# mj-will/aspire

Measured on AMD Instinct MI355X. Metric: particle-steps/sec (N x n_steps), 1M particles d=32; log-evidence err vs ref, higher is better.
Workload: dtype f64

## Files before the change

### aspire_amd/csrc/asmc_common.h

```cpp
#pragma once
#include <hip/hip_runtime.h>
#include <stdint.h>
#include <stdio.h>
#include <string.h>

#include "../../include/asmc.h"

#define ASMC_WAVE 64
#define ASMC_BLOCK 256
#define ASMC_MAX_BLOCKS 2048
#define ASMC_SCAN_TILE 2048
#define ASMC_PCN_MAX_GRID (1 << 20)
#define ASMC_GAMMA_BATCH 8
#define ASMC_MAX_PCN_STEPS 2048
#define BM_SC_N 256
#define BM_LG_N 128
#define BM_TAB_N (BM_SC_N + BM_LG_N)

void asmc_set_error(const char* fmt, ...);
void asmc_bm_table_host(double* tab);
struct asmc_ctx;
int asmc_count_nonfinite_enqueue(asmc_ctx* ctx, int64_t n, const double* v, hipStream_t st);
unsigned long long* asmc_count_slot(asmc_ctx* ctx);
struct asmc_ctx;
// ... 30 lines not shown
            return ASMC_ERR_ARG;                                  \
        }                                                         \
    } while (0)

#define ASMC_LAUNCH_CHECK()                                                                 \
    do {                                                                                    \
        hipError_t _e = hipGetLastError();                                                  \
        if (_e != hipSuccess) {                                                             \
            asmc_set_error("kernel launch failed: %s (%s:%d)", hipGetErrorString(_e),       \
                           __FILE__, __LINE__);                                             \
            return ASMC_ERR_HIP;                                                            \
        }                                                                                   \
    } while (0)

#define ASMC_TILECTR_BYTES ((sizeof(unsigned int) * (2 * ASMC_MAX_PCN_STEPS + 4) + 255) / 256 * 256)
struct asmc_ctx {
    int device;
    int64_t n_max;
    int d_max;
    int num_cu;
    double* d_partials;
    double* d_small;
    unsigned long long* d_keys;
    double* d_tiles;
    long long* d_tiles_i;
    double* d_gram;
    unsigned int* d_guide;
    unsigned char* d_flags;
    double* d_gamma;
    int64_t gam_n;
// ... 22 lines not shown
    long long* d_counts;
    double* d_rho;
    unsigned long long* d_stretch;
    unsigned long long* d_mh;
    unsigned int* d_tilectr;
    unsigned int* d_bar;
    unsigned int bar_base[17];
    unsigned long long flow_nonfinite;
    int poison_lds;
    int isw_disabled;
    unsigned long long* d_pcgtab;
    long long* d_select;
    unsigned long long ptab_tag, ysplit_seq;
    double* d_ptab;
    double* d_bmtab;
    double* d_mmtab;
    double* d_f16tab;
    size_t f16tab_bytes;
    int (*count_hook)(void*, asmc_stream);
    void* count_hook_user;
    long long* count_cell;
    int count_cells;
    int64_t count_n_global;
    int mutate_defer, mutate_pending_steps;
    hipEvent_t ev_mutate;
    hipEvent_t ev_is;
    int is_result_pending;
    unsigned long long lq_nan;
    void* rccl_allreduce;
    void* rccl_comm;
// ... 83 lines not shown
```

### aspire_amd/csrc/asmc_ctx.hip

```cpp
#include <dlfcn.h>
#include <stdarg.h>

#include <math.h>

#include "asmc_common.h"

static thread_local char g_err[512] = "";

void asmc_set_error(const char* fmt, ...) {
    va_list ap;
    va_start(ap, fmt);
    vsnprintf(g_err, sizeof(g_err), fmt, ap);
    va_end(ap);
}

__global__ __launch_bounds__(256) void k_poison_lds(int words) {
    extern __shared__ unsigned int s_poison[];
    for (int i = threadIdx.x; i < words; i += 256) s_poison[i] = 0xFFFFFFFFu;
    __syncthreads();
    if (s_poison[(threadIdx.x * 977) % words] != 0xFFFFFFFFu) __builtin_trap();
}
void asmc_poison_lds(asmc_ctx* ctx, hipStream_t st) {
    const int bytes = 160 * 1024 - 1024;
    static bool attr_set_dev[ASMC_MAX_DEVICES] = {false}; bool& attr_set = attr_set_dev[asmc_dev_slot(ctx)];
// ... 170 lines not shown
    const size_t student = (size_t)d_max * (d_max + 1) + (size_t)(ASMC_STUDENT_MAX_ROWS / 64) * (d_max + 2);
    dmalloc((void**)&c->d_student, sizeof(double) * student);
    if (e == hipSuccess) e = hipHostMalloc((void**)&c->h_student, sizeof(double) * student, hipHostMallocDefault);
    dmalloc((void**)&c->d_counts, sizeof(long long) * (size_t)(ASMC_MAX_PCN_STEPS + ASMC_MAX_BLOCKS + n_max / 64 + 8));
    dmalloc((void**)&c->d_rho, sizeof(double) * (ASMC_MAX_PCN_STEPS + 8));
    dmalloc((void**)&c->d_stretch, sizeof(unsigned long long) * ASMC_MAX_PCN_STEPS);
    dmalloc((void**)&c->d_mh, sizeof(unsigned long long) * ASMC_MAX_PCN_STEPS);
    if (e == hipSuccess) e = hipMemset(c->d_tilectr, 0, ASMC_TILECTR_BYTES);
    dmalloc((void**)&c->d_bar, sizeof(unsigned int) * 1024 * 17);
    if (e == hipSuccess) e = hipMemset(c->d_bar, 0, sizeof(unsigned int) * 1024 * 17);
    dmalloc((void**)&c->d_pcgtab, sizeof(unsigned long long) * (64 * 4 + 8));
    dmalloc((void**)&c->d_select, sizeof(long long) * (2 * (ASMC_SELECT_THREADS / 64) + 8));
    dmalloc((void**)&c->d_ptab, sizeof(double) * (2 * 32 * 32 + 32 + 3 * ASMC_MAX_COMPONENTS * (1 + 2 * 32) + 64));
    dmalloc((void**)&c->d_bmtab, sizeof(double) * 2 * BM_TAB_N);
    dmalloc((void**)&c->d_ref, sizeof(double) * (128 + 128 * 128));
    if (e == hipSuccess) {
        double tab[2 * BM_TAB_N];
        asmc_bm_table_host(tab);
        e = hipMemcpy(c->d_bmtab, tab, sizeof(tab), hipMemcpyHostToDevice);
    }
    if (e == hipSuccess) e = hipHostMalloc((void**)&c->h_pinned, sizeof(double) * 8192, hipHostMallocDefault);
    if (e == hipSuccess) e = hipHostMalloc((void**)&c->h_gram, sizeof(double) * (128 + 128 * 128), hipHostMallocDefault);
    if (e != hipSuccess) {
        asmc_set_error("asmc_ctx_create: allocation failed: %s", hipGetErrorString(e));
        asmc_ctx_destroy(c);
        return ASMC_ERR_NOMEM;
    }
    *ctx_out = c;
    return ASMC_OK;
}
// ... 15 lines not shown
    if (c->h_student) (void)hipHostFree(c->h_student);
    if (c->d_ysoa) (void)hipFree(c->d_ysoa);
    if (c->d_xpad) (void)hipFree(c->d_xpad);
    (void)hipFree(c->d_counts);
    (void)hipFree(c->d_rho);
    (void)hipFree(c->d_stretch);
    (void)hipFree(c->d_mh);
    (void)hipFree(c->d_tilectr);
    (void)hipFree(c->d_rec);
    (void)hipFree(c->d_bar);
    (void)hipFree(c->d_pcgtab);
    (void)hipFree(c->d_select);
    (void)hipFree(c->d_ptab);
    (void)hipFree(c->d_bmtab);
    (void)hipFree(c->d_ref);
    if (c->prof_ev) {
        for (int i = 0; i < 2 * ASMC_PROF_MAX; i++) (void)hipEventDestroy(c->prof_ev[i]);
        delete[] c->prof_ev;
        delete[] c->prof_label;
    }
    if (c->h_pinned) (void)hipHostFree(c->h_pinned);
    if (c->h_gram) (void)hipHostFree(c->h_gram);
    if (c->ev_mutate) (void)hipEventDestroy(c->ev_mutate);
    if (c->ev_is) (void)hipEventDestroy(c->ev_is);
    delete c;
    return ASMC_OK;
}

}
```

### aspire_amd/csrc/asmc_flow_dev.h

```cpp
#pragma once
#include "asmc_common.h"

typedef float floatx16 __attribute__((ext_vector_type(16)));


__device__ __forceinline__ float flow_standardise(float x, float loc, float scale, float rcp) {
    const float a = x - loc;
    const float q0 = a * rcp;
    const float r = fmaf(-scale, q0, a);
    return fmaf(r, rcp, q0);
}

typedef float flow_std2 __attribute__((ext_vector_type(2)));
__device__ __forceinline__ flow_std2 flow_standardise2(flow_std2 x, flow_std2 loc, flow_std2 scale, flow_std2 rcp) {
    const flow_std2 a = x - loc;
    const flow_std2 q0 = a * rcp;
    const flow_std2 r = __builtin_elementwise_fma(-scale, q0, a);
    return __builtin_elementwise_fma(r, rcp, q0);
}

template <bool INVERSE>
__device__ __forceinline__ void flow_affine(float& x, float sraw, float t, float& ladj, int form) {
    if (form == 0) {
        const float sv = 2.0f - 4.0f * __builtin_amdgcn_rcpf(__expf(sraw) + 1.0f);
// ... 594 lines not shown
                for (int nb = 0; nb < NBM; nb++) ah[nb] = ahn[nb], al[nb] = aln[nb];
            } else {
                a_load(g + 1, ah, al);
            }
            __builtin_amdgcn_sched_barrier(0);
        }
    }
    flow_f2 lacc = {0.0f, 0.0f};
#pragma unroll
    for (int q = 0; q < H / 2; q += 2)
        flow_affine2<false>(trans[q], trans[q + 1], o[q / 16][q % 16], o[(q + 1) / 16][(q + 1) % 16], o[(H / 2 + q) / 16][(H / 2 + q) % 16],
                            o[(H / 2 + q + 1) / 16][(H / 2 + q + 1) % 16], lacc, FORM >= 0 ? FORM : form);
    ladj += lacc.x + lacc.y;
}

template <int H, int W, int THREADS>
__device__ __forceinline__ void flow_stage_hs(float* __restrict__ sp, const float* __restrict__ packed, int n_layers) {
    using FD = FlowDims<H, W>;
    constexpr int L4 = FD::LAYER / 4, B4 = FD::BIAS / 4;
    const int total4 = n_layers * L4;
    for (int i4 = threadIdx.x; i4 < total4; i4 += THREADS) {
        const int in_layer = i4 % L4;
        if (in_layer < B4) {
            reinterpret_cast<float4*>(sp)[i4] = reinterpret_cast<const float4*>(packed)[i4];
            continue;
        }
        const int local = in_layer - B4;
        if ((local / 64) & 1) continue;
        const float4 f0 = reinterpret_cast<const float4*>(packed)[i4], f1 = reinterpret_cast<const float4*>(packed)[i4 + 64];
        const float xv[8] = {f0.x, f0.y, f0.z, f0.w, f1.x, f1.y, f1.z, f1.w};
        half8 hi, lo;
        float wmax = 0.0f;
        split8_f16<false>(xv, hi, lo, wmax);
        reinterpret_cast<half8*>(sp)[i4] = hi;
        reinterpret_cast<half8*>(sp)[i4 + 64] = lo;
    }
}
```

### aspire_amd/csrc/asmc_pcn.hip

```cpp
#include <stdlib.h>

#include <chrono>

#include "asmc_common.h"
#include "asmc_tile.h"
#include "asmc_pcn_dev.h"
#include "asmc_transform_dev.h"

template <typename T>
__device__ __forceinline__ double mixture_eval(const MixDev& m, int d, const char* row) {
    double best = -INFINITY;
    double terms[ASMC_MAX_COMPONENTS];
    const int C = m.C;
    for (int c = 0; c < C; c++) {
        double q = 0.0;
        const double* mu = m.mu + (size_t)c * d;
        const double* pr = m.prec + (size_t)c * d;
        for (int j = 0; j < d; j++) {
            const double t = row_get<T>(row, j) - mu[j];
            q = fma(t * t, pr[j], q);
        }
        const double v = m.logw[c] - 0.5 * q;
        terms[c] = v;
        best = fmax(best, v);
// ... 2921 lines not shown
            pc.noise = ASMC_NOISE_F64;
            if (prm->x_dtype == ASMC_F64)
                return launch_pcn_step<double, 0>(ctx, n, (double*)x, ll, lp, lq, pc, d_rho, 0, d_block, &grid, nullptr, nullptr, nullptr, st);
            return launch_pcn_step<float, 0>(ctx, n, (float*)x, ll, lp, lq, pc, d_rho, 0, d_block, &grid, nullptr, nullptr, nullptr, st);
        };
        rc = convert(PCN_WHITEN);
        if (rc) return rc;
        const bool fused = soa && asmc_pcn_flow_fused_ok(prm, flow);
        if (d_noise > 0 && !fused) {
            asmc_set_error("asmc_pcn_mutate_flow: the zero-padded form needs the one-kernel step");
            return ASMC_ERR_UNSUPPORTED;
        }
        if (fused) {
            ASMC_HIP(hipMemsetAsync(ctx->d_tilectr, 0, ASMC_TILECTR_BYTES + ((size_t)((n + 63) / 64) + 15) / 16 * 16, st));
            pd.tile_par = ctx->d_flags;
        }
        for (int t = 0; t < (fused ? n_steps : 0); t++) {
            const uint32_t step = step0 + (uint32_t)t;
            rc = pcn_prepare_gamma(ctx, n, pd, step, st);
            if (rc) return rc;
            PcnAdaptArgs ad = {ctx->d_tilectr + ASMC_MAX_PCN_STEPS + t,
                               reinterpret_cast<unsigned long long*>(ctx->d_tilectr + 2 * ASMC_MAX_PCN_STEPS),
                               ctx->count_hook ? ctx->count_cell : nullptr,
                               ctx->count_hook && t > 0 ? ctx->count_cell : nullptr, d_counts, d_rho, d_rho_hist,
                               prm->target_accept, ctx->count_hook ? ctx->count_n_global : n, t, prm->adapt, t == n_steps - 1};
            const int lag = prm->adapt >= 2 ? prm->adapt : 1;
            if (ctx->count_hook && lag > ctx->count_cells) {
                asmc_set_error("adapt_lag %d needs %d exchange cells, the installed hook has %d (asmc_pcn_set_count_cells)", lag, lag, ctx->count_cells);
                return ASMC_ERR_ARG;
            }
// ... 344 lines not shown
```

### aspire_amd/csrc/asmc_pcn_dev.h

```cpp
#pragma once
#include "asmc_common.h"

bool asmc_flow_math_split();

struct PcnAdaptArgs {
    unsigned int* done;
    unsigned long long* nonfinite;
    long long* cell;
    const long long* prev_cell;
    long long* counts_out;
    double* rho;
    double* rho_hist;
    double target;
    int64_t n;
    int t, adapt;
    int last;
};

__device__ __forceinline__ double pcn_adapt_rho(double rho, long long c, int64_t n, double target, int t) {
    const double acc = (double)c / (double)n;
    double r = exp(log(rho) + (acc - target) / pow((double)(t + 1), 0.75));
    r = r < 1e-4 ? 1e-4 : r;
    r = r > 0.99 ? 0.99 : r;
    return r;
// ... 344 lines not shown
        return (double)__uint_as_float(v);
    }
}
template <typename T>
__device__ __forceinline__ void soa_store(__amdgpu_buffer_rsrc_t r, unsigned voff, unsigned soff, double x) {
    if constexpr (sizeof(T) == 8) {
        using u2 = decltype(__builtin_amdgcn_raw_buffer_load_b64(r, 0, 0, 0));
        __builtin_amdgcn_raw_buffer_store_b64(__builtin_bit_cast(u2, x), r, (int)voff, (int)soff, 0);
    } else {
        __builtin_amdgcn_raw_buffer_store_b32(__float_as_uint((float)x), r, (int)voff, (int)soff, 0);
    }
}


bool asmc_pcn_flow_fused_ok(const asmc_pcn_params* prm, const asmc_coupling* f);
int asmc_pcn_flow_fused_launch(asmc_ctx* ctx, int64_t n, int x_dtype, double* ll, double* lp, double* lq, const PcnDev& pd,
                               const asmc_coupling* f, const double* rho_ptr, uint32_t step, unsigned int* tile_counter,
                               long long* block_counts, int* grid_out, const PcnAdaptArgs& adapt, hipStream_t st);

#define MM_WHITEN 0
#define MM_STEP 1
#define MM_UNWHITEN 2
#define MM_STEP_T 3
#define MM_XPROPOSE 4
#define MM_XPROPOSE_T 5
#define MM_UNWHITEN_X 6
bool asmc_pcn_mm_supported(int d, const void* x);
int asmc_pcn_mm_pack(asmc_ctx* ctx, const PcnDev& pd, hipStream_t st);
int asmc_pcn_flow16_tables(asmc_ctx* ctx, const PcnDev& pd, const asmc_coupling* f, hipStream_t st);
int asmc_pcn_flow16_launch(asmc_ctx* ctx, int64_t n, int x_dtype, void* x, double* ll, double* lp, double* lq, const PcnDev& pd,
// ... 9 lines not shown
```

### aspire_amd/csrc/asmc_pcn_fused.hip

```cpp
#include <stdlib.h>

#include "asmc_common.h"
#include <type_traits>
#include "asmc_pcn_dev.h"
#include "asmc_flow_dev.h"

#ifndef FUSED_THREADS
#define FUSED_THREADS 512
#endif

#define FUSED_TL_DOUBLES 1368
#define FUSED_MAX_COMPONENTS 4
#ifndef MV_DEPTH
#define MV_DEPTH 4
#endif
typedef double double2v __attribute__((ext_vector_type(2)));
__host__ __device__ constexpr int mv_group(int bi) {
    int g = 0;
    while ((g + 1) * (g + 2) <= bi) g++;
    return g;
}
template <int I, int N, typename F>
__device__ __forceinline__ void mv_for_each(F& f) {
    if constexpr (I < N) {
// ... 16 lines not shown
    y = __builtin_bit_cast(double, ((unsigned long long)hi[1] << 32) | lo[1]);
}
__device__ __forceinline__ void fused_swap16(double& x, double& y) {
    const unsigned long long xb = __builtin_bit_cast(unsigned long long, x), yb = __builtin_bit_cast(unsigned long long, y);
    const auto lo = __builtin_amdgcn_permlane16_swap((unsigned)xb, (unsigned)yb, false, false);
    const auto hi = __builtin_amdgcn_permlane16_swap((unsigned)(xb >> 32), (unsigned)(yb >> 32), false, false);
    x = __builtin_bit_cast(double, ((unsigned long long)hi[0] << 32) | lo[0]);
    y = __builtin_bit_cast(double, ((unsigned long long)hi[1] << 32) | lo[1]);
}
__device__ __forceinline__ void fused_transpose4(double& q0, double& q1, double& q2, double& q3) {
    fused_swap32(q0, q2);
    fused_swap32(q1, q3);
    fused_swap16(q0, q1);
    fused_swap16(q2, q3);
}
#ifndef HS1P_PREFETCH
#define HS1P_PREFETCH false
#endif
#ifndef FUSED_PRIO_A
#define FUSED_PRIO_A 2
#define FUSED_PRIO_B 1
#endif
#ifndef MV_CHUNK
#define MV_CHUNK 8
#endif
template <typename T, int W, int NOISE, bool HS, int KIND = ASMC_FLOW_COUPLING, bool MIX = false>
__global__ __launch_bounds__(FUSED_THREADS) void k_pcn_flow_fused(
    int64_t n, double* __restrict__ ll, double* __restrict__ lp, double* __restrict__ lq, const double* __restrict__ ptab,
    PcnScalars p, const double* rho_ptr, uint32_t step, const float* __restrict__ packed, int n_layers,
    const float* __restrict__ loc, const float* __restrict__ scale, float ladj0, float base_const,
    unsigned int* __restrict__ tile_counter, long long* __restrict__ block_counts, PcnAdaptArgs ad, int par_words, int affine) {
    constexpr int D = 32, H = 16, THREADS = FUSED_THREADS;
    constexpr int HF = KIND == ASMC_FLOW_MAF ? 32 : H;
    static_assert(KIND == ASMC_FLOW_COUPLING || HS, "the autoregressive variant runs the split-fp16 layers only");
    using FD = FlowDims<HF, W>;
    extern __shared__ __align__(16) float sp[];
    if (HS) {
        flow_stage_hs<HF, W, THREADS>(sp, packed, n_layers);
    } else {
        const int total4 = n_layers * FD::LAYER / 4;
        for (int base = 0; base < total4; base += THREADS * 8) {
            float4 tmp[8];
#pragma unroll
            for (int q = 0; q < 8; q++) {
                const int i4 = base + q * THREADS + threadIdx.x;
                tmp[q] = i4 < total4 ? reinterpret_cast<const float4*>(packed)[i4] : make_float4(0.f, 0.f, 0.f, 0.f);
            }
#pragma unroll
            for (int q = 0; q < 8; q++) {
                const int i4 = base + q * THREADS + threadIdx.x;
                if (i4 < total4) reinterpret_cast<float4*>(sp)[i4] = tmp[q];
            }
        }
    }
    double* tl = reinterpret_cast<double*>(sp + (size_t)n_layers * FD::LAYER);
    constexpr int T_MU = D * D, T_LLMU = T_MU + D, T_LLPR = T_LLMU + D, T_LPMU = T_LLPR + D, T_LPPR = T_LPMU + D,
                  T_LOGW = T_LPPR + D, T_LOC = T_LOGW + 2;
    static_assert(T_LOC + 3 * D / 2 <= FUSED_TL_DOUBLES, "pCN tables");
    constexpr int M_MU = 12 * 64, M_MIX = M_MU + D, M_LOGW = M_MIX + 2 * FUSED_MAX_COMPONENTS * 2 * D, M_LOC = M_LOGW + 2 * FUSED_MAX_COMPONENTS;
    static_assert(M_LOC + 3 * D / 2 <= FUSED_TL_DOUBLES, "pCN tables (matrix-core variant)");
    constexpr bool MVM = FUSED_MVMFMA && FUSED_INPLACE;
    {
        const double* m0g = ptab + 2 * PTAB_TRI(D) + D;
        const int dr = (p.d_noise > 0 && p.d_noise < D) ? p.d_noise : D;
        const int dhalf = KIND == ASMC_FLOW_MAF ? 16 : dr / 2;
        auto nat = [&](int r) -> int {
            const int c = r < 16 ? (r < dhalf ? r : -1) : (r - 16 + dhalf);
            return (c >= 0 && c < dr) ? c : -1;
        };
        if (MVM) {
            for (int e = threadIdx.x; e < 12 * 64; e += THREADS) {
                const int slot = e >> 6, l = e & 63, mb = slot < 4 ? 0 : 1, sidx = slot < 4 ? slot : slot - 4;
                const int i = l & 15, j = nat(16 * mb + 4 * (i & 3) + (i >> 2)), k = 4 * sidx + (l >> 4);
                tl[e] = (j >= 0 && k <= j) ? ptab[j * (j + 1) / 2 + k] : 0.0;
            }
            for (int e = threadIdx.x; e < D; e += THREADS) {
                const int j = nat(16 * ((e >> 2) & 1) + 4 * (e >> 3) + (e & 3));
                tl[M_MU + e] = j >= 0 ? ptab[2 * PTAB_TRI(D) + j] : 0.0;
                reinterpret_cast<float*>(tl + M_LOC)[e] = j >= 0 ? loc[j] : 0.0f;
                reinterpret_cast<float*>(tl + M_LOC)[D + e] = j >= 0 ? scale[j] : 1.0f;
                reinterpret_cast<float*>(tl + M_LOC)[2 * D + e] = j >= 0 ? 1.0f / scale[j] : 1.0f;
            }
            for (int e = threadIdx.x; e < 2 * FUSED_MAX_COMPONENTS * D; e += THREADS) {
                const int tc = e / D, er = e % D, tt = tc / FUSED_MAX_COMPONENTS, c = tc % FUSED_MAX_COMPONENTS;
                const int j = nat(16 * ((er >> 2) & 1) + 4 * (er >> 3) + (er & 3));
                const bool live = j >= 0 && c < (tt == 0 ? p.c_ll : p.c_lp);
                const double* mg = m0g + (size_t)tt * PTAB_MIX(D);
                tl[M_MIX + tc * 2 * D + er] = live ? mg[ASMC_MAX_COMPONENTS + c * D + j] : 0.0;
                tl[M_MIX + tc * 2 * D + D + er] = live ? mg[ASMC_MAX_COMPONENTS * (1 + D) + c * D + j] : 0.0;
            }
            if (threadIdx.x < 2 * FUSED_MAX_COMPONENTS) {
                const int tt = threadIdx.x / FUSED_MAX_COMPONENTS, c = threadIdx.x % FUSED_MAX_COMPONENTS;
                tl[M_LOGW + threadIdx.x] = c < (tt == 0 ? p.c_ll : p.c_lp) ? m0g[(size_t)tt * PTAB_MIX(D) + c] : -INFINITY;
            }
        } else {
            for (int e = threadIdx.x; e < D * D; e += THREADS) {
                const int j = e / D, k = e - j * D;
                tl[e] = k <= j ? ptab[j * (j + 1) / 2 + k] : 0.0;
            }
            for (int e = threadIdx.x; e < D; e += THREADS) {
                tl[T_MU + e] = ptab[2 * PTAB_TRI(D) + e];
                tl[T_LLMU + e] = m0g[ASMC_MAX_COMPONENTS + e];
                tl[T_LLPR + e] = m0g[ASMC_MAX_COMPONENTS * (1 + D) + e];
                tl[T_LPMU + e] = m0g[PTAB_MIX(D) + ASMC_MAX_COMPONENTS + e];
                tl[T_LPPR + e] = m0g[PTAB_MIX(D) + ASMC_MAX_COMPONENTS * (1 + D) + e];
                reinterpret_cast<float*>(tl + T_LOC)[e] = loc[e];
                reinterpret_cast<float*>(tl + T_LOC)[D + e] = scale[e];
                reinterpret_cast<float*>(tl + T_LOC)[2 * D + e] = 1.0f / scale[e];
            }
        }
        if (!MVM && threadIdx.x == 0) tl[T_LOGW] = m0g[0], tl[T_LOGW + 1] = m0g[PTAB_MIX(D)];
    }
    bm_d2* bmt = reinterpret_cast<bm_d2*>(tl + FUSED_TL_DOUBLES);
    if (NOISE == ASMC_NOISE_F64) bm_tab_stage<THREADS>(bmt, p.bmtab);
    unsigned* const par_bits = reinterpret_cast<unsigned*>(bmt + BM_TAB_N);
    for (int wd = threadIdx.x; wd < par_words; wd += THREADS) {
        const uint4 b0 = reinterpret_cast<const uint4*>(p.tile_par)[2 * wd], b1 = reinterpret_cast<const uint4*>(p.tile_par)[2 * wd + 1];
        const unsigned q[8] = {b0.x, b0.y, b0.z, b0.w, b1.x, b1.y, b1.z, b1.w};
        unsigned bits = 0;
#pragma unroll
        for (int k = 0; k < 8; k++) {
            const unsigned nib = (((q[k] & 0x01010101u) * 0x01020408u) >> 24) & 0xFu;
            bits |= nib << (4 * k);
        }
        par_bits[wd] = bits;
    }
    __syncthreads();
    const int lane = threadIdx.x & 63, wave = threadIdx.x >> 6, hh = lane >> 5;
    const bool first_on_simd = __builtin_amdgcn_readfirstlane(wave) < 4;
#ifdef FUSED_STAGGER
    if (!first_on_simd) {
#pragma unroll 1
        for (int i = 0; i < FUSED_STAGGER; i++) __builtin_amdgcn_s_sleep(127);
    }
#endif
    double rho;
    if (ad.prev_cell) {
        const double rp = ad.rho_hist[ad.t - 1];
        if (ad.adapt <= 1) {
            const long long cp = *ad.prev_cell;
            rho = ad.adapt ? pcn_adapt_rho(rp, cp, ad.n, ad.target, ad.t - 1) : rp;
            if (blockIdx.x == 0 && threadIdx.x == 0) ad.counts_out[ad.t - 1] = cp;
        } else if (ad.t % ad.adapt == 0) {
            double r = rp;
            for (int tp = ad.t - ad.adapt; tp < ad.t; tp++) {
                const long long ct = ad.prev_cell[tp % ad.adapt];
                r = pcn_adapt_rho(r, ct, ad.n, ad.target, tp);
                if (blockIdx.x == 0 && threadIdx.x == 0) ad.counts_out[tp] = ct;
            }
            rho = r;
// ... 71 lines not shown
        const bool valid = i < n;
        const unsigned ys_tile = t * 64u * (unsigned)sizeof(T);
        const __amdgpu_buffer_rsrc_t ysr = __builtin_amdgcn_make_buffer_rsrc(par ? ysu1 : ysu, 0, half_records, 0x00020000);
        (void)valid;
#pragma unroll
        for (int j = 0; j < D; j++) v[j] = soa_load<T>(ysr, ys_lane, ys_tile + (unsigned)j * ys_row);
        oll = olp = olq = 0.0;
        if (valid) oll = ll[i], olp = lp[i], olq = lq[i];
    };
    double v[D];
    double oll = 0.0, olp = 0.0, olq = 0.0;
    unsigned t = idle_wave ? 0xFFFFFFFFu : (unsigned)__builtin_amdgcn_readfirstlane((int)tile_fetch());
    unsigned par = 0;
    bool have = (int64_t)t < n_tiles;
    if (have) {
        par = tile_parity(t);
        tile_load(t, par, v, oll, olp, olq);
    }
    while (have) {
        STAMP(0);
        int zoff;
        asm volatile("v_mov_b32 %0, 0" : "=v"(zoff));
        const double* __restrict__ Lt = tl + zoff;
        const float* __restrict__ locs = reinterpret_cast<const float*>(tl + (MVM ? M_LOC : T_LOC)) + zoff;
        const int64_t i = (int64_t)t * 64 + lane;
        const bool valid = i < n;
        const unsigned ys_tile = t * 64u * (unsigned)sizeof(T);
#if !FUSED_INPLACE
        const __amdgpu_buffer_rsrc_t ypr = __builtin_amdgcn_make_buffer_rsrc(par ? ysu : ysu1, 0, half_records, 0x00020000);
#endif
        const unsigned long long gid = p.gid0 + (unsigned long long)i;
        double q0 = 0.0, q1 = 0.0, q0t = 0.0;
        if (p.gam != nullptr) {
// ... 484 lines not shown
#endif
#ifndef FUSED_NOSB
        __builtin_amdgcn_sched_barrier(0);
#endif
        t = tn, par = par_n, have = have_n;
        oll = olln, olp = olpn, olq = olqn;
#pragma unroll
        for (int j = 0; j < D; j++) v[j] = vn[j];
    }
#ifdef FUSED_STAMP
    if (lane == 0 && blockIdx.x == 7 && (wave == 0 || wave == 4) && ntile > 0)
        printf("wave %d tiles %d | fetch %llu yload %llu noise %llu matvec %llu park+swap %llu flowA %llu flowB %llu accept %llu (cycles per tile)\n", wave, ntile,
               tsum[0] / ntile, tsum[1] / ntile, tsum[2] / ntile, tsum[3] / ntile, tsum[4] / ntile, tsum[5] / ntile, tsum[6] / ntile, tsum[7] / ntile);
#endif
    __shared__ long long s_cnt[THREADS / 64];
    n_acc = wave_sum_ll(n_acc);
    n_bad = wave_sum_ll(n_bad);
    if (lane == 0 && n_bad != 0 && ad.nonfinite) atomicAdd(ad.nonfinite, (unsigned long long)n_bad);
    if (lane == 0) s_cnt[wave] = n_acc;
    __syncthreads();
    if (threadIdx.x == 0) {
        long long tsum = 0;
        for (int w = 0; w < THREADS / 64; w++) tsum += s_cnt[w];
        block_counts[blockIdx.x] = tsum;
    }
    if (ad.done == nullptr) return;
    __shared__ int s_last;
    if (threadIdx.x == 0) {
        __builtin_amdgcn_fence(__ATOMIC_RELEASE, "agent");
        const unsigned int tk = __hip_atomic_fetch_add(ad.done, 1u, __ATOMIC_RELAXED, __HIP_MEMORY_SCOPE_AGENT);
        s_last = (tk == gridDim.x - 1u);
        if (s_last) __builtin_amdgcn_fence(__ATOMIC_ACQUIRE, "agent");
// ... 56 lines not shown
#define ASMC_FUSED_CASE_K(WW, NZ, HSV, KD) ASMC_FUSED_CASE_KM(WW, NZ, HSV, KD, false)
#define ASMC_FUSED_CASE_KM(WW, NZ, HSV, KD, MX)                                                                           \
    if (f->hidden == WW && pd.noise == NZ && hs == HSV && f->kind == KD && mix == MX) {                                   \
        auto kern = k_pcn_flow_fused<T, WW, NZ, HSV, KD, MX>;                                                                 \
        const size_t lds0 = (size_t)f->n_layers * FlowDims<(KD == ASMC_FLOW_MAF ? 32 : 16), WW>::LAYER * sizeof(float) + FUSED_TL_DOUBLES * sizeof(double) + BM_TAB_N * sizeof(bm_d2); \
        const size_t par_bytes = (size_t)((n_tiles + 31) / 32) * 4;    \
        const int par_words = (!FUSED_INPLACE && lds0 + par_bytes <= 160 * 1024) ? (int)(par_bytes / 4) : 0;                     \
        const size_t lds = lds0 + (size_t)par_words * 4;                                                                     \
        static size_t attr_lds_dev[ASMC_MAX_DEVICES] = {0}; size_t& attr_lds = attr_lds_dev[asmc_dev_slot(ctx)];                                                                                      \
        if (lds > 64 * 1024 && lds > attr_lds) {                                                                         \
            ASMC_HIP(hipFuncSetAttribute(reinterpret_cast<const void*>(kern), hipFuncAttributeMaxDynamicSharedMemorySize, (int)lds)); \
            attr_lds = lds;                                                                                              \
        }                                                                                                                \
        ASMC_LAUNCH(ctx, st, "k_pcn_flow_fused", kern, dim3(grid), dim3(FUSED_THREADS), lds, st, n, ll, lp, lq,                     \
                    (const double*)ctx->d_ptab, ps, rho_ptr, step, f->packed_dev, (int)f->n_layers, f->loc_dev, f->scale_dev, \
                    ladj0, base_const, tile_counter, block_counts, adapt, par_words, KD == ASMC_FLOW_MAF ? (int)f->affine : 0);  \
        ASMC_LAUNCH_CHECK();                                                                                             \
        return ASMC_OK;                                                                                                  \
    }
#define ASMC_FUSED_CASE(WW, NZ, HSV) ASMC_FUSED_CASE_K(WW, NZ, HSV, ASMC_FLOW_COUPLING)
    ASMC_FUSED_CASE(64, ASMC_NOISE_F64, true)
#ifndef FUSED_ONLY_HEADLINE
    ASMC_FUSED_CASE_KM(64, ASMC_NOISE_F64, true, ASMC_FLOW_COUPLING, true)
    ASMC_FUSED_CASE_KM(64, ASMC_NOISE_F32, true, ASMC_FLOW_COUPLING, true)
    ASMC_FUSED_CASE(64, ASMC_NOISE_F64, false)
    ASMC_FUSED_CASE(64, ASMC_NOISE_F32, true)
    ASMC_FUSED_CASE(64, ASMC_NOISE_F32, false)
    ASMC_FUSED_CASE(32, ASMC_NOISE_F64, true)
    ASMC_FUSED_CASE(32, ASMC_NOISE_F64, false)
    ASMC_FUSED_CASE(32, ASMC_NOISE_F32, true)
    ASMC_FUSED_CASE(32, ASMC_NOISE_F32, false)
// ... 21 lines not shown
    const bool mvm = FUSED_MVMFMA && FUSED_INPLACE && f->kind == ASMC_FLOW_COUPLING && f->hidden == 64 && asmc_flow_math_split();
    const int cmax = mvm ? FUSED_MAX_COMPONENTS : 1;
    if (prm->log_likelihood.n_components < 1 || prm->log_likelihood.n_components > cmax) return false;
    if (prm->log_prior.n_components < 1 || prm->log_prior.n_components > cmax) return false;
    if (!(f->hidden == 32 || f->hidden == 64 || f->hidden == 128)) return false;
    if (f->kind == ASMC_FLOW_MAF) {
        if (!asmc_flow_math_split() || f->hidden == 128) return false;
        const size_t per_tr = (size_t)((2 * (f->hidden / 32) + 2) * 32 + f->hidden * 32 + f->hidden * f->hidden + 2 * 32 * f->hidden) * sizeof(float);
        return per_tr * (size_t)f->n_layers + FUSED_TL_DOUBLES * sizeof(double) + BM_TAB_N * sizeof(bm_d2) <= 160 * 1024;
    }
    const size_t per_layer = (size_t)((2 * (f->hidden / 32) + 1) * 32 + f->hidden * 16 + f->hidden * f->hidden + 2 * 16 * f->hidden) * sizeof(float);
    return per_layer * (size_t)f->n_layers + FUSED_TL_DOUBLES * sizeof(double) + BM_TAB_N * sizeof(bm_d2) <= 160 * 1024;
}


int asmc_pcn_flow_fused_launch(asmc_ctx* ctx, int64_t n, int x_dtype, double* ll, double* lp, double* lq, const PcnDev& pd,
                               const asmc_coupling* f, const double* rho_ptr, uint32_t step, unsigned int* tile_counter,
                               long long* block_counts, int* grid_out, const PcnAdaptArgs& adapt, hipStream_t st) {
    if (x_dtype == ASMC_F64)
        return launch_pcn_flow_fused<double>(ctx, n, ll, lp, lq, pd, f, rho_ptr, step, tile_counter, block_counts, grid_out, adapt, st);
    return launch_pcn_flow_fused<float>(ctx, n, ll, lp, lq, pd, f, rho_ptr, step, tile_counter, block_counts, grid_out, adapt, st);
}
```

Before: 3.626 billion.

## Prebuild fused pCN LDS image once per run and bulk-copy it per block

Moves the per-block construction of the LDS image (flow weights with fp16 split, pCN tables, Box-Muller table) into a separate kernel that writes a global image buffer once per sampler call. Each fused-step block then bulk-copies that image with buffer loads after issuing its first tile load, so the setup overlaps with the initial tile fetch. The change also merges two wave reductions into one DPP-based pass and reads tile parity via readfirstlane. The cost is an extra 160KB device buffer, an added kernel launch, and reliance on the image staying valid across all steps.

Measured after the change: 3.622 billion (median of 2 runs). About the same (-0.1%).

```diff
diff --git a/aspire_amd/csrc/asmc_common.h b/aspire_amd/csrc/asmc_common.h
--- a/aspire_amd/csrc/asmc_common.h
+++ b/aspire_amd/csrc/asmc_common.h
@@ -68,6 +68,7 @@
     } while (0)
 
 #define ASMC_TILECTR_BYTES ((sizeof(unsigned int) * (2 * ASMC_MAX_PCN_STEPS + 4) + 255) / 256 * 256)
+#define ASMC_FUSED_IMG_BYTES (160 * 1024)
 struct asmc_ctx {
     int device;
     int64_t n_max;
@@ -120,6 +121,7 @@
     unsigned long long ptab_tag, ysplit_seq;
     double* d_ptab;
     double* d_bmtab;
+    float* d_fusedimg;
     double* d_mmtab;
     double* d_f16tab;
     size_t f16tab_bytes;
diff --git a/aspire_amd/csrc/asmc_ctx.hip b/aspire_amd/csrc/asmc_ctx.hip
--- a/aspire_amd/csrc/asmc_ctx.hip
+++ b/aspire_amd/csrc/asmc_ctx.hip
@@ -208,6 +208,8 @@
     dmalloc((void**)&c->d_ptab, sizeof(double) * (2 * 32 * 32 + 32 + 3 * ASMC_MAX_COMPONENTS * (1 + 2 * 32) + 64));
     dmalloc((void**)&c->d_bmtab, sizeof(double) * 2 * BM_TAB_N);
     dmalloc((void**)&c->d_ref, sizeof(double) * (128 + 128 * 128));
+    dmalloc((void**)&c->d_fusedimg, ASMC_FUSED_IMG_BYTES);
+    if (e == hipSuccess) e = hipMemset(c->d_fusedimg, 0, ASMC_FUSED_IMG_BYTES);
     if (e == hipSuccess) {
         double tab[2 * BM_TAB_N];
         asmc_bm_table_host(tab);
@@ -253,6 +255,7 @@
     (void)hipFree(c->d_ptab);
     (void)hipFree(c->d_bmtab);
     (void)hipFree(c->d_ref);
+    (void)hipFree(c->d_fusedimg);
     if (c->prof_ev) {
         for (int i = 0; i < 2 * ASMC_PROF_MAX; i++) (void)hipEventDestroy(c->prof_ev[i]);
         delete[] c->prof_ev;
diff --git a/aspire_amd/csrc/asmc_flow_dev.h b/aspire_amd/csrc/asmc_flow_dev.h
--- a/aspire_amd/csrc/asmc_flow_dev.h
+++ b/aspire_amd/csrc/asmc_flow_dev.h
@@ -632,12 +632,12 @@
     ladj += lacc.x + lacc.y;
 }
 
-template <int H, int W, int THREADS>
-__device__ __forceinline__ void flow_stage_hs(float* __restrict__ sp, const float* __restrict__ packed, int n_layers) {
+template <int H, int W>
+__device__ __forceinline__ void flow_stage_hs_at(float* __restrict__ sp, const float* __restrict__ packed, int n_layers, const int tid, const int nthr) {
     using FD = FlowDims<H, W>;
     constexpr int L4 = FD::LAYER / 4, B4 = FD::BIAS / 4;
     const int total4 = n_layers * L4;
-    for (int i4 = threadIdx.x; i4 < total4; i4 += THREADS) {
+    for (int i4 = tid; i4 < total4; i4 += nthr) {
         const int in_layer = i4 % L4;
         if (in_layer < B4) {
             reinterpret_cast<float4*>(sp)[i4] = reinterpret_cast<const float4*>(packed)[i4];
@@ -654,3 +654,7 @@
         reinterpret_cast<half8*>(sp)[i4 + 64] = lo;
     }
 }
+template <int H, int W, int THREADS>
+__device__ __forceinline__ void flow_stage_hs(float* __restrict__ sp, const float* __restrict__ packed, int n_layers) {
+    flow_stage_hs_at<H, W>(sp, packed, n_layers, (int)threadIdx.x, THREADS);
+}
diff --git a/aspire_amd/csrc/asmc_pcn.hip b/aspire_amd/csrc/asmc_pcn.hip
--- a/aspire_amd/csrc/asmc_pcn.hip
+++ b/aspire_amd/csrc/asmc_pcn.hip
@@ -2959,6 +2959,8 @@
         if (fused) {
             ASMC_HIP(hipMemsetAsync(ctx->d_tilectr, 0, ASMC_TILECTR_BYTES + ((size_t)((n + 63) / 64) + 15) / 16 * 16, st));
             pd.tile_par = ctx->d_flags;
+            rc = asmc_pcn_flow_fused_image(ctx, pd, flow, st);
+            if (rc) return rc;
         }
         for (int t = 0; t < (fused ? n_steps : 0); t++) {
             const uint32_t step = step0 + (uint32_t)t;
diff --git a/aspire_amd/csrc/asmc_pcn_dev.h b/aspire_amd/csrc/asmc_pcn_dev.h
--- a/aspire_amd/csrc/asmc_pcn_dev.h
+++ b/aspire_amd/csrc/asmc_pcn_dev.h
@@ -382,6 +382,7 @@
 
 
 bool asmc_pcn_flow_fused_ok(const asmc_pcn_params* prm, const asmc_coupling* f);
+int asmc_pcn_flow_fused_image(asmc_ctx* ctx, const PcnDev& pd, const asmc_coupling* f, hipStream_t st);
 int asmc_pcn_flow_fused_launch(asmc_ctx* ctx, int64_t n, int x_dtype, double* ll, double* lp, double* lq, const PcnDev& pd,
                                const asmc_coupling* f, const double* rho_ptr, uint32_t step, unsigned int* tile_counter,
                                long long* block_counts, int* grid_out, const PcnAdaptArgs& adapt, hipStream_t st);
diff --git a/aspire_amd/csrc/asmc_pcn_fused.hip b/aspire_amd/csrc/asmc_pcn_fused.hip
--- a/aspire_amd/csrc/asmc_pcn_fused.hip
+++ b/aspire_amd/csrc/asmc_pcn_fused.hip
@@ -54,6 +54,15 @@
     fused_swap16(q0, q1);
     fused_swap16(q2, q3);
 }
+__device__ __forceinline__ void fused_wave_sum2(long long& c0, long long& c1) {
+    int a = (int)c0, b = (int)c1;
+    a += __builtin_amdgcn_update_dpp(0, a, 0xB1, 0xF, 0xF, false), b += __builtin_amdgcn_update_dpp(0, b, 0xB1, 0xF, 0xF, false);
+    a += __builtin_amdgcn_update_dpp(0, a, 0x4E, 0xF, 0xF, false), b += __builtin_amdgcn_update_dpp(0, b, 0x4E, 0xF, 0xF, false);
+    a += __builtin_amdgcn_update_dpp(0, a, 0x141, 0xF, 0xF, false), b += __builtin_amdgcn_update_dpp(0, b, 0x141, 0xF, 0xF, false);
+    a += __builtin_amdgcn_update_dpp(0, a, 0x140, 0xF, 0xF, false), b += __builtin_amdgcn_update_dpp(0, b, 0x140, 0xF, 0xF, false);
+    c0 = (long long)__builtin_amdgcn_readlane(a, 0) + __builtin_amdgcn_readlane(a, 16) + __builtin_amdgcn_readlane(a, 32) + __builtin_amdgcn_readlane(a, 48);
+    c1 = (long long)__builtin_amdgcn_readlane(b, 0) + __builtin_amdgcn_readlane(b, 16) + __builtin_amdgcn_readlane(b, 32) + __builtin_amdgcn_readlane(b, 48);
+}
 #ifndef HS1P_PREFETCH
 #define HS1P_PREFETCH false
 #endif
@@ -64,41 +73,49 @@
 #ifndef MV_CHUNK
 #define MV_CHUNK 8
 #endif
-template <typename T, int W, int NOISE, bool HS, int KIND = ASMC_FLOW_COUPLING, bool MIX = false>
-__global__ __launch_bounds__(FUSED_THREADS) void k_pcn_flow_fused(
-    int64_t n, double* __restrict__ ll, double* __restrict__ lp, double* __restrict__ lq, const double* __restrict__ ptab,
-    PcnScalars p, const double* rho_ptr, uint32_t step, const float* __restrict__ packed, int n_layers,
-    const float* __restrict__ loc, const float* __restrict__ scale, float ladj0, float base_const,
-    unsigned int* __restrict__ tile_counter, long long* __restrict__ block_counts, PcnAdaptArgs ad, int par_words, int affine) {
-    constexpr int D = 32, H = 16, THREADS = FUSED_THREADS;
-    constexpr int HF = KIND == ASMC_FLOW_MAF ? 32 : H;
-    static_assert(KIND == ASMC_FLOW_COUPLING || HS, "the autoregressive variant runs the split-fp16 layers only");
+#ifndef FUSED_STAGE_INKERNEL
+#define FUSED_STAGE_INKERNEL 0
+#endif
+#ifndef FUSED_COPY_BATCH
+#define FUSED_COPY_BATCH 10
+#endif
+struct FusedTab {
+    static constexpr int D = 32;
+    static constexpr int T_MU = D * D, T_LLMU = T_MU + D, T_LLPR = T_LLMU + D, T_LPMU = T_LLPR + D, T_LPPR = T_LPMU + D,
+                         T_LOGW = T_LPPR + D, T_LOC = T_LOGW + 2;
+    static constexpr int M_MU = 12 * 64, M_MIX = M_MU + D, M_LOGW = M_MIX + 2 * FUSED_MAX_COMPONENTS * 2 * D, M_LOC = M_LOGW + 2 * FUSED_MAX_COMPONENTS;
+};
+static_assert(FusedTab::T_LOC + 3 * FusedTab::D / 2 <= FUSED_TL_DOUBLES, "pCN tables");
+static_assert(FusedTab::M_LOC + 3 * FusedTab::D / 2 <= FUSED_TL_DOUBLES, "pCN tables (matrix-core variant)");
+template <int W, int NOISE, bool HS, int KIND>
+__device__ __forceinline__ void fused_stage_image(float* __restrict__ sp, const int tid, const int nthr, const double* __restrict__ ptab,
+                                                  const PcnScalars& p, const float* __restrict__ packed, int n_layers,
+                                                  const float* __restrict__ loc, const float* __restrict__ scale) {
+    constexpr int D = FusedTab::D;
+    constexpr int HF = KIND == ASMC_FLOW_MAF ? 32 : 16;
     using FD = FlowDims<HF, W>;
-    extern __shared__ __align__(16) float sp[];
     if (HS) {
-        flow_stage_hs<HF, W, THREADS>(sp, packed, n_layers);
+        flow_stage_hs_at<HF, W>(sp, packed, n_layers, tid, nthr);
     } else {
         const int total4 = n_layers * FD::LAYER / 4;
-        for (int base = 0; base < total4; base += THREADS * 8) {
+        for (int base = 0; base < total4; base += nthr * 8) {
             float4 tmp[8];
 #pragma unroll
             for (int q = 0; q < 8; q++) {
-                const int i4 = base + q * THREADS + threadIdx.x;
+                const int i4 = base + q * nthr + tid;
                 tmp[q] = i4 < total4 ? reinterpret_cast<const float4*>(packed)[i4] : make_float4(0.f, 0.f, 0.f, 0.f);
             }
 #pragma unroll
             for (int q = 0; q < 8; q++) {
-                const int i4 = base + q * THREADS + threadIdx.x;
+                const int i4 = base + q * nthr + tid;
                 if (i4 < total4) reinterpret_cast<float4*>(sp)[i4] = tmp[q];
             }
         }
     }
     double* tl = reinterpret_cast<double*>(sp + (size_t)n_layers * FD::LAYER);
-    constexpr int T_MU = D * D, T_LLMU = T_MU + D, T_LLPR = T_LLMU + D, T_LPMU = T_LLPR + D, T_LPPR = T_LPMU + D,
-                  T_LOGW = T_LPPR + D, T_LOC = T_LOGW + 2;
-    static_assert(T_LOC + 3 * D / 2 <= FUSED_TL_DOUBLES, "pCN tables");
-    constexpr int M_MU = 12 * 64, M_MIX = M_MU + D, M_LOGW = M_MIX + 2 * FUSED_MAX_COMPONENTS * 2 * D, M_LOC = M_LOGW + 2 * FUSED_MAX_COMPONENTS;
-    static_assert(M_LOC + 3 * D / 2 <= FUSED_TL_DOUBLES, "pCN tables (matrix-core variant)");
+    constexpr int T_MU = FusedTab::T_MU, T_LLMU = FusedTab::T_LLMU, T_LLPR = FusedTab::T_LLPR, T_LPMU = FusedTab::T_LPMU, T_LPPR = FusedTab::T_LPPR,
+                  T_LOGW = FusedTab::T_LOGW, T_LOC = FusedTab::T_LOC, M_MU = FusedTab::M_MU, M_MIX = FusedTab::M_MIX, M_LOGW = FusedTab::M_LOGW,
+                  M_LOC = FusedTab::M_LOC;
     constexpr bool MVM = FUSED_MVMFMA && FUSED_INPLACE;
     {
         const double* m0g = ptab + 2 * PTAB_TRI(D) + D;
@@ -109,19 +126,19 @@
             return (c >= 0 && c < dr) ? c : -1;
         };
         if (MVM) {
-            for (int e = threadIdx.x; e < 12 * 64; e += THREADS) {
+            for (int e = tid; e < 12 * 64; e += nthr) {
                 const int slot = e >> 6, l = e & 63, mb = slot < 4 ? 0 : 1, sidx = slot < 4 ? slot : slot - 4;
                 const int i = l & 15, j = nat(16 * mb + 4 * (i & 3) + (i >> 2)), k = 4 * sidx + (l >> 4);
                 tl[e] = (j >= 0 && k <= j) ? ptab[j * (j + 1) / 2 + k] : 0.0;
             }
-            for (int e = threadIdx.x; e < D; e += THREADS) {
+            for (int e = tid; e < D; e += nthr) {
                 const int j = nat(16 * ((e >> 2) & 1) + 4 * (e >> 3) + (e & 3));
                 tl[M_MU + e] = j >= 0 ? ptab[2 * PTAB_TRI(D) + j] : 0.0;
                 reinterpret_cast<float*>(tl + M_LOC)[e] = j >= 0 ? loc[j] : 0.0f;
                 reinterpret_cast<float*>(tl + M_LOC)[D + e] = j >= 0 ? scale[j] : 1.0f;
                 reinterpret_cast<float*>(tl + M_LOC)[2 * D + e] = j >= 0 ? 1.0f / scale[j] : 1.0f;
             }
-            for (int e = threadIdx.x; e < 2 * FUSED_MAX_COMPONENTS * D; e += THREADS) {
+            for (int e = tid; e < 2 * FUSED_MAX_COMPONENTS * D; e += nthr) {
                 const int tc = e / D, er = e % D, tt = tc / FUSED_MAX_COMPONENTS, c = tc % FUSED_MAX_COMPONENTS;
                 const int j = nat(16 * ((er >> 2) & 1) + 4 * (er >> 3) + (er & 3));
                 const bool live = j >= 0 && c < (tt == 0 ? p.c_ll : p.c_lp);
@@ -129,16 +146,16 @@
                 tl[M_MIX + tc * 2 * D + er] = live ? mg[ASMC_MAX_COMPONENTS + c * D + j] : 0.0;
                 tl[M_MIX + tc * 2 * D + D + er] = live ? mg[ASMC_MAX_COMPONENTS * (1 + D) + c * D + j] : 0.0;
             }
-            if (threadIdx.x < 2 * FUSED_MAX_COMPONENTS) {
-                const int tt = threadIdx.x / FUSED_MAX_COMPONENTS, c = threadIdx.x % FUSED_MAX_COMPONENTS;
-                tl[M_LOGW + threadIdx.x] = c < (tt == 0 ? p.c_ll : p.c_lp) ? m0g[(size_t)tt * PTAB_MIX(D) + c] : -INFINITY;
+            if (tid < 2 * FUSED_MAX_COMPONENTS) {
+                const int tt = tid / FUSED_MAX_COMPONENTS, c = tid % FUSED_MAX_COMPONENTS;
+                tl[M_LOGW + tid] = c < (tt == 0 ? p.c_ll : p.c_lp) ? m0g[(size_t)tt * PTAB_MIX(D) + c] : -INFINITY;
             }
         } else {
-            for (int e = threadIdx.x; e < D * D; e += THREADS) {
+            for (int e = tid; e < D * D; e += nthr) {
                 const int j = e / D, k = e - j * D;
                 tl[e] = k <= j ? ptab[j * (j + 1) / 2 + k] : 0.0;
             }
-            for (int e = threadIdx.x; e < D; e += THREADS) {
+            for (int e = tid; e < D; e += nthr) {
                 tl[T_MU + e] = ptab[2 * PTAB_TRI(D) + e];
                 tl[T_LLMU + e] = m0g[ASMC_MAX_COMPONENTS + e];
                 tl[T_LLPR + e] = m0g[ASMC_MAX_COMPONENTS * (1 + D) + e];
@@ -149,31 +166,43 @@
                 reinterpret_cast<float*>(tl + T_LOC)[2 * D + e] = 1.0f / scale[e];
             }
         }
-        if (!MVM && threadIdx.x == 0) tl[T_LOGW] = m0g[0], tl[T_LOGW + 1] = m0g[PTAB_MIX(D)];
+        if (!MVM && tid == 0) tl[T_LOGW] = m0g[0], tl[T_LOGW + 1] = m0g[PTAB_MIX(D)];
     }
     bm_d2* bmt = reinterpret_cast<bm_d2*>(tl + FUSED_TL_DOUBLES);
-    if (NOISE == ASMC_NOISE_F64) bm_tab_stage<THREADS>(bmt, p.bmtab);
+    if (NOISE == ASMC_NOISE_F64)
+        for (int e = tid; e < BM_TAB_N; e += nthr) bmt[e] = reinterpret_cast<const bm_d2*>(p.bmtab)[e];
+}
+__host__ __device__ constexpr size_t fused_image_bytes(int n_layers, int layer_floats, int noise) {
+    return (size_t)n_layers * layer_floats * sizeof(float) + FUSED_TL_DOUBLES * sizeof(double) + (noise == ASMC_NOISE_F64 ? BM_TAB_N * sizeof(bm_d2) : 0);
+}
+template <int W, int NOISE, bool HS, int KIND>
+__global__ __launch_bounds__(FUSED_THREADS) void k_fused_image(float* __restrict__ img, const double* __restrict__ ptab, PcnScalars p,
+                                                               const float* __restrict__ packed, int n_layers, const float* __restrict__ loc,
+                                                               const float* __restrict__ scale) {
+    fused_stage_image<W, NOISE, HS, KIND>(img, (int)(blockIdx.x * FUSED_THREADS + threadIdx.x), (int)(gridDim.x * FUSED_THREADS), ptab, p, packed,
+                                          n_layers, loc, scale);
+}
+template <typename T, int W, int NOISE, bool HS, int KIND = ASMC_FLOW_COUPLING, bool MIX = false>
+__global__ __launch_bounds__(FUSED_THREADS) void k_pcn_flow_fused(
+    int64_t n, double* __restrict__ ll, double* __restrict__ lp, double* __restrict__ lq, const double* __restrict__ ptab,
+    PcnScalars p, const double* rho_ptr, uint32_t step, const float* __restrict__ packed, int n_layers,
+    const float* __restrict__ loc, const float* __restrict__ scale, float ladj0, float base_const,
+    unsigned int* __restrict__ tile_counter, long long* __restrict__ block_counts, PcnAdaptArgs ad, int par_words, int affine,
+    const float4* __restrict__ img, int img4) {
+    constexpr int D = 32, H = 16, THREADS = FUSED_THREADS;
+    constexpr int HF = KIND == ASMC_FLOW_MAF ? 32 : H;
+    static_assert(KIND == ASMC_FLOW_COUPLING || HS, "the autoregressive variant runs the split-fp16 layers only");
+    using FD = FlowDims<HF, W>;
+    extern __shared__ __align__(16) float sp[];
+    double* tl = reinterpret_cast<double*>(sp + (size_t)n_layers * FD::LAYER);
+    constexpr int T_LOGW = FusedTab::T_LOGW, T_LOC = FusedTab::T_LOC, T_MU = FusedTab::T_MU, T_LLMU = FusedTab::T_LLMU, T_LLPR = FusedTab::T_LLPR,
+                  T_LPMU = FusedTab::T_LPMU, T_LPPR = FusedTab::T_LPPR, M_MU = FusedTab::M_MU, M_MIX = FusedTab::M_MIX, M_LOGW = FusedTab::M_LOGW,
+                  M_LOC = FusedTab::M_LOC;
+    constexpr bool MVM = FUSED_MVMFMA && FUSED_INPLACE;
+    bm_d2* bmt = reinterpret_cast<bm_d2*>(tl + FUSED_TL_DOUBLES);
     unsigned* const par_bits = reinterpret_cast<unsigned*>(bmt + BM_TAB_N);
-    for (int wd = threadIdx.x; wd < par_words; wd += THREADS) {
-        const uint4 b0 = reinterpret_cast<const uint4*>(p.tile_par)[2 * wd], b1 = reinterpret_cast<const uint4*>(p.tile_par)[2 * wd + 1];
-        const unsigned q[8] = {b0.x, b0.y, b0.z, b0.w, b1.x, b1.y, b1.z, b1.w};
-        unsigned bits = 0;
-#pragma unroll
-        for (int k = 0; k < 8; k++) {
-            const unsigned nib = (((q[k] & 0x01010101u) * 0x01020408u) >> 24) & 0xFu;
-            bits |= nib << (4 * k);
-        }
-        par_bits[wd] = bits;
-    }
-    __syncthreads();
-    const int lane = threadIdx.x & 63, wave = threadIdx.x >> 6, hh = lane >> 5;
-    const bool first_on_simd = __builtin_amdgcn_readfirstlane(wave) < 4;
-#ifdef FUSED_STAGGER
-    if (!first_on_simd) {
-#pragma unroll 1
-        for (int i = 0; i < FUSED_STAGGER; i++) __builtin_amdgcn_s_sleep(127);
-    }
-#endif
+    const int lane = threadIdx.x & 63, wave = __builtin_amdgcn_readfirstlane((int)(threadIdx.x >> 6)), hh = lane >> 5;
+    const bool first_on_simd = wave < 4;
     double rho;
     if (ad.prev_cell) {
         const double rp = ad.rho_hist[ad.t - 1];
@@ -275,9 +304,50 @@
     unsigned par = 0;
     bool have = (int64_t)t < n_tiles;
     if (have) {
-        par = tile_parity(t);
+        par = FUSED_INPLACE ? 0u : (unsigned)__builtin_amdgcn_readfirstlane((int)tile_par[t]);
         tile_load(t, par, v, oll, olp, olq);
     }
+#if FUSED_STAGE_INKERNEL
+    fused_stage_image<W, NOISE, HS, KIND>(sp, (int)threadIdx.x, THREADS, ptab, p, packed, n_layers, loc, scale);
+#else
+    {
+        static_assert(2 * FUSED_COPY_BATCH * THREADS * 16 == ASMC_FUSED_IMG_BYTES, "two batches cover the image buffer, and no load leaves it");
+        const __amdgpu_buffer_rsrc_t imr = __builtin_amdgcn_make_buffer_rsrc(const_cast<float4*>(img), 0, img4 * 16, 0x00020000);
+        using img_u4 = decltype(__builtin_amdgcn_raw_buffer_load_b128(imr, 0, 0, 0));
+#pragma unroll
+        for (int b = 0; b < 2; b++) {
+            const int base = b * THREADS * FUSED_COPY_BATCH;
+            if (base >= img4) break;
+            img_u4 tmp[FUSED_COPY_BATCH];
+#pragma unroll
+            for (int q = 0; q < FUSED_COPY_BATCH; q++)
+                tmp[q] = __builtin_amdgcn_raw_buffer_load_b128(imr, (int)threadIdx.x * 16, (base + q * THREADS) * 16, 0);
+#pragma unroll
+            for (int q = 0; q < FUSED_COPY_BATCH; q++) {
+                const int i4 = base + q * THREADS + (int)threadIdx.x;
+                if (i4 < img4) reinterpret_cast<img_u4*>(sp)[i4] = tmp[q];
+            }
+        }
+    }
+#endif
+    for (int wd = threadIdx.x; wd < par_words; wd += THREADS) {
+        const uint4 b0 = reinterpret_cast<const uint4*>(p.tile_par)[2 * wd], b1 = reinterpret_cast<const uint4*>(p.tile_par)[2 * wd + 1];
+        const unsigned q[8] = {b0.x, b0.y, b0.z, b0.w, b1.x, b1.y, b1.z, b1.w};
+        unsigned bits = 0;
+#pragma unroll
+        for (int k = 0; k < 8; k++) {
+            const unsigned nib = (((q[k] & 0x01010101u) * 0x01020408u) >> 24) & 0xFu;
+            bits |= nib << (4 * k);
+        }
+        par_bits[wd] = bits;
+    }
+    __syncthreads();
+#ifdef FUSED_STAGGER
+    if (!first_on_simd) {
+#pragma unroll 1
+        for (int i = 0; i < FUSED_STAGGER; i++) __builtin_amdgcn_s_sleep(127);
+    }
+#endif
     while (have) {
         STAMP(0);
         int zoff;
@@ -792,8 +862,7 @@
                tsum[0] / ntile, tsum[1] / ntile, tsum[2] / ntile, tsum[3] / ntile, tsum[4] / ntile, tsum[5] / ntile, tsum[6] / ntile, tsum[7] / ntile);
 #endif
     __shared__ long long s_cnt[THREADS / 64];
-    n_acc = wave_sum_ll(n_acc);
-    n_bad = wave_sum_ll(n_bad);
+    fused_wave_sum2(n_acc, n_bad);
     if (lane == 0 && n_bad != 0 && ad.nonfinite) atomicAdd(ad.nonfinite, (unsigned long long)n_bad);
     if (lane == 0) s_cnt[wave] = n_acc;
     __syncthreads();
@@ -880,7 +949,8 @@
         }                                                                                                                \
         ASMC_LAUNCH(ctx, st, "k_pcn_flow_fused", kern, dim3(grid), dim3(FUSED_THREADS), lds, st, n, ll, lp, lq,                     \
                     (const double*)ctx->d_ptab, ps, rho_ptr, step, f->packed_dev, (int)f->n_layers, f->loc_dev, f->scale_dev, \
-                    ladj0, base_const, tile_counter, block_counts, adapt, par_words, KD == ASMC_FLOW_MAF ? (int)f->affine : 0);  \
+                    ladj0, base_const, tile_counter, block_counts, adapt, par_words, KD == ASMC_FLOW_MAF ? (int)f->affine : 0,    \
+                    (const float4*)ctx->d_fusedimg, FUSED_STAGE_INKERNEL ? 0 : (int)(fused_image_bytes((int)f->n_layers, FlowDims<(KD == ASMC_FLOW_MAF ? 32 : 16), WW>::LAYER, NZ) / 16)); \
         ASMC_LAUNCH_CHECK();                                                                                             \
         return ASMC_OK;                                                                                                  \
     }
@@ -932,6 +1002,52 @@
 }
 
 
+int asmc_pcn_flow_fused_image(asmc_ctx* ctx, const PcnDev& pd, const asmc_coupling* f, hipStream_t st) {
+#if FUSED_STAGE_INKERNEL
+    return ASMC_OK;
+#else
+    PcnScalars ps;
+    memset(&ps, 0, sizeof(ps));
+    ps.d_noise = pd.d_noise;
+    ps.c_ll = pd.ll.C;
+    ps.c_lp = pd.lp.C;
+    ps.bmtab = pd.bmtab;
+    const bool hs = asmc_flow_math_split();
+#define ASMC_FUSED_IMAGE_CASE(WW, NZ, HSV, KD)                                                                                       \
+    if (f->hidden == WW && pd.noise == NZ && hs == HSV && f->kind == KD) {                                                           \
+        constexpr int LAYER = FlowDims<(KD == ASMC_FLOW_MAF ? 32 : 16), WW>::LAYER;                                                  \
+        static_assert(LAYER % 4 == 0 && (FUSED_TL_DOUBLES * sizeof(double)) % 16 == 0, "the image is copied in 16-byte pieces");     \
+        ASMC_REQUIRE(fused_image_bytes((int)f->n_layers, LAYER, NZ) <= ASMC_FUSED_IMG_BYTES, "the step's LDS image exceeds its buffer"); \
+        const int grid = (int)(((size_t)f->n_layers * LAYER / 4 + FUSED_THREADS - 1) / FUSED_THREADS);   \
+        ASMC_LAUNCH(ctx, st, "k_fused_image", (k_fused_image<WW, NZ, HSV, KD>), dim3(grid), dim3(FUSED_THREADS), 0, st, ctx->d_fusedimg, \
+                    (const double*)ctx->d_ptab, ps, f->packed_dev, (int)f->n_layers, f->loc_dev, f->scale_dev);                      \
+        ASMC_LAUNCH_CHECK();                                                                                                         \
+        return ASMC_OK;                                                                                                              \
+    }
+    ASMC_FUSED_IMAGE_CASE(64, ASMC_NOISE_F64, true, ASMC_FLOW_COUPLING)
+#ifndef FUSED_ONLY_HEADLINE
+    ASMC_FUSED_IMAGE_CASE(64, ASMC_NOISE_F32, true, ASMC_FLOW_COUPLING)
+    ASMC_FUSED_IMAGE_CASE(64, ASMC_NOISE_F64, false, ASMC_FLOW_COUPLING)
+    ASMC_FUSED_IMAGE_CASE(64, ASMC_NOISE_F32, false, ASMC_FLOW_COUPLING)
+    ASMC_FUSED_IMAGE_CASE(32, ASMC_NOISE_F64, true, ASMC_FLOW_COUPLING)
+    ASMC_FUSED_IMAGE_CASE(32, ASMC_NOISE_F32, true, ASMC_FLOW_COUPLING)
+    ASMC_FUSED_IMAGE_CASE(32, ASMC_NOISE_F64, false, ASMC_FLOW_COUPLING)
+    ASMC_FUSED_IMAGE_CASE(32, ASMC_NOISE_F32, false, ASMC_FLOW_COUPLING)
+    ASMC_FUSED_IMAGE_CASE(128, ASMC_NOISE_F64, true, ASMC_FLOW_COUPLING)
+    ASMC_FUSED_IMAGE_CASE(128, ASMC_NOISE_F32, true, ASMC_FLOW_COUPLING)
+    ASMC_FUSED_IMAGE_CASE(128, ASMC_NOISE_F64, false, ASMC_FLOW_COUPLING)
+    ASMC_FUSED_IMAGE_CASE(128, ASMC_NOISE_F32, false, ASMC_FLOW_COUPLING)
+    ASMC_FUSED_IMAGE_CASE(64, ASMC_NOISE_F64, true, ASMC_FLOW_MAF)
+    ASMC_FUSED_IMAGE_CASE(64, ASMC_NOISE_F32, true, ASMC_FLOW_MAF)
+    ASMC_FUSED_IMAGE_CASE(32, ASMC_NOISE_F64, true, ASMC_FLOW_MAF)
+    ASMC_FUSED_IMAGE_CASE(32, ASMC_NOISE_F32, true, ASMC_FLOW_MAF)
+#endif
+#undef ASMC_FUSED_IMAGE_CASE
+    asmc_set_error("fused flow step: unsupported flow (kind %d, hidden width %d)", (int)f->kind, (int)f->hidden);
+    return ASMC_ERR_UNSUPPORTED;
+#endif
+}
+
 int asmc_pcn_flow_fused_launch(asmc_ctx* ctx, int64_t n, int x_dtype, double* ll, double* lp, double* lq, const PcnDev& pd,
                                const asmc_coupling* f, const double* rho_ptr, uint32_t step, unsigned int* tile_counter,
                                long long* block_counts, int* grid_out, const PcnAdaptArgs& adapt, hipStream_t st) {
```
